# dafyddstephenson/ucla-roms

Hardware: AMD Instinct MI355X
Metric: grid-cell-updates/sec (higher is better)
Workload: dtype f64; 1 GPU; C3: basin 1024x1024x100, NONLIN+SPLIT EOS, T+S, LMD KPP/BKPP/RIMIX/NONLOCAL, dt=300s, ndtfast=60 (nfast=82); NT=2, nfast=82, parallelism=domain decomposition 1x1, halo_transport=none (single rank), fast_exchange_interval=1, exchange_order=none (single rank), s2d_window=True, comm_bootstrap=none (single rank)

## Files before the change

### include/roms_gpu.h

```cpp
#ifndef ROMS_GPU_H
#define ROMS_GPU_H

#ifdef __cplusplus
extern "C" {
#endif

#define ROMS_GPU_ABI_VERSION 22
#define ROMS_MAX_FAST 288

typedef struct roms_dims {
  int Lm, Mm, N, NT;
  int LLm, MMm;
  int np_xi, np_eta, inode, jnode;
  int iSW_corn, jSW_corn;
  int ew_periodic, ns_periodic;
  int west_exchng, east_exchng, south_exchng, north_exchng;
} roms_dims;

#define ROMS_LMD_MIXING   1
#define ROMS_LMD_KPP      2
#define ROMS_LMD_BKPP     4
#define ROMS_LMD_RIMIX    8
#define ROMS_LMD_CONVEC   16
#define ROMS_LMD_NONLOCAL 32
#define ROMS_LMD_ALL      63
#define ROMS_LMD_ICELAND  47
#define ROMS_LMD_DDMIX    64

typedef struct roms_cfg {
  int nonlin_eos;
// ... 101 lines not shown
} roms_case;
int roms_gpu_init_case(const roms_case *c, int device, roms_tlev *t);
int roms_gpu_init_case_comm(const roms_case *c, int np_xi, int np_eta, void *comm, int device, roms_tlev *t);

int roms_gpu_comm_unique_id(void *id128);
int roms_gpu_comm_create(const void *id128, int nranks, int rank, int device, void **comm);
int roms_gpu_comm_create_local(int group, int nranks, int rank, void **comm);
typedef int (*roms_host_allgather_fn)(void *ctx, const void *send, long nbytes, void *recv);
int roms_gpu_comm_create_host(int nranks, int rank, int device, roms_host_allgather_fn allgather, void *ctx,
                              void **comm);
int roms_gpu_comm_destroy(void *comm);
int roms_gpu_halo_transport(void);
int roms_gpu_halo_exchanges(long *per_step, int *fast_interval);
int roms_gpu_halo_overlap(void);
int roms_gpu_s2d_window(void);
#define ROMS_COLPATH_SEG 1
#define ROMS_COLPATH_GLOBAL 2
int roms_gpu_column_path(void);
int roms_gpu_kpp_lean(void);
int roms_gpu_vgrid(void);
int roms_gpu_vgrid2(void);
int roms_gpu_vgrid_check(long out[3]);
int roms_gpu_tracer_pair(long launches[2]);
int roms_gpu_horizontal_path(int out[8]);
int roms_gpu_selftest_zero_fill(long n, int chunks, long *bad);
int roms_gpu_halo_plan(int Lm, int Mm, int np_xi, int np_eta, int inode, int jnode, int ew_periodic,
                       int ns_periodic, int peer[8], long count[8], int strip[4]);
long roms_gpu_halo_map(int Lm, int Mm, int np_xi, int np_eta, int inode, int jnode, int ew_periodic,
                       int ns_periodic, int dir, int unpack, int *i, int *j, long cap);
long roms_gpu_halo_map_wide(int Lm, int Mm, int np_xi, int np_eta, int inode, int jnode, int ew_periodic,
                            int ns_periodic, int width, int dir, int unpack, int *i, int *j, long cap);

#define ROMS_FRC_SURFACE 1
#define ROMS_FRC_BRY     2
int roms_gpu_frc_record(int field_id, int slot, double rec_time, const double *data);
int roms_gpu_frc_interp(double modtime, int kinds);
int roms_gpu_frc_clock(double start_time, int on);
int roms_gpu_set_tide_data(int ntides, const double *ftide, const double *pot_re, const double *pot_im,
                           const double *ztide_re, const double *ztide_im, const double *utide_re,
                           const double *utide_im, const double *vtide_re, const double *vtide_im);
int roms_gpu_set_tides(double time);

#define ROMS_WRT_Z    1
#define ROMS_WRT_UB   2
#define ROMS_WRT_VB   4
#define ROMS_WRT_U    8
// ... 40 lines not shown
```

### ucla-roms_amd/csrc/k_common.h

```cpp
#pragma once
#include "roms_dev.h"
#include <type_traits>

namespace roms {

constexpr unsigned kBufOff = 0x80000000u;
struct BufF64 {
  __amdgpu_buffer_rsrc_t r;
  __device__ __forceinline__ explicit BufF64(const double* p, long n = 0)
      : r(__builtin_amdgcn_make_buffer_rsrc(const_cast<double*>(p), (short)0,
                                            n > 0 ? (int)(unsigned)(n * 8) : (int)0x7fffffff, 0x00020000)) {}
  __device__ __forceinline__ double ld(unsigned vb, unsigned sb) const {
    return __builtin_bit_cast(double, __builtin_amdgcn_raw_buffer_load_b64(r, (int)vb, (int)sb, 0));
  }
  __device__ __forceinline__ void st(double v, unsigned vb, unsigned sb) const {
    __builtin_amdgcn_raw_buffer_store_b64(__builtin_bit_cast(__attribute__((ext_vector_type(2))) int, v), r, (int)vb,
                                          (int)sb, 0);
  }
};

constexpr int kUVW = kBX + 4, kUVH = kBY + 4, kUVN = kUVW * kUVH;

struct ColLds {
  double* p;
// ... 173 lines not shown
  const double Fl = a.fu(m, j);
  if (upstream) {
    const double cm = el[1] - el[0], c0 = el[2] - el[1];
    return 0.5 * (a.t(m, j) + a.t(m - 1, j)) * Fl - 0.1666666666666666 * (cm * fmax0(Fl) + c0 * fmin0(Fl));
  }
  const double gm = 0.5 * (el[1] + el[0]), g0 = 0.5 * (el[2] + el[1]);
  return 0.5 * (a.t(m, j) + a.t(m - 1, j) - 0.3333333333333333 * (g0 - gm)) * Fl;
}
template <class A>
__device__ __forceinline__ double tracer_fe(const Bounds& b, const A& a, int i, int m, bool upstream) {
  const int lo = b.south_edge ? b.jstr : -1000000, hi = b.north_edge ? b.jend + 1 : 1000000;
  double el[3];
  for (int q = 0; q < 3; q++) {
    const int p = iclamp(m - 1 + q, lo, hi);
    el[q] = (a.t(i, p) - a.t(i, p - 1)) * a.vm(i, p);
  }
  const double Fl = a.fv(i, m);
  if (upstream) {
    const double cm = el[1] - el[0], c0 = el[2] - el[1];
    return 0.5 * (a.t(i, m) + a.t(i, m - 1)) * Fl - 0.1666666666666666 * (cm * fmax0(Fl) + c0 * fmin0(Fl));
  }
  const double gm = 0.5 * (el[1] + el[0]), g0 = 0.5 * (el[2] + el[1]);
  return 0.5 * (a.t(i, m) + a.t(i, m - 1) - 0.3333333333333333 * (g0 - gm)) * Fl;
}

struct TracerWin {
  double T[kUVN], UM[kUVN], VM[kUVN], FU[kUVN], FV[kUVN];
};
__device__ __forceinline__ void tracer_win_fill(const Bounds& b, const Fields& F, TracerWin& W, int ib, int jb,
                                                long kk, const double* T) {
  for (int q = threadIdx.x + kBX * threadIdx.y; q < kUVN; q += kBX * kBY) {
    const int i = ib + q % kUVW, j = jb + q / kUVW;
    if (i < -1 || i > b.Lm + 2 || j < -1 || j > b.Mm + 2) continue;
    const long o = IJ(b, i, j);
    if (T) {
      W.T[q] = T[o + kk];
    } else {
      W.UM[q] = F.umask[o];
      W.VM[q] = F.vmask[o];
      W.FU[q] = F.FlxU[o + kk];
      W.FV[q] = F.FlxV[o + kk];
    }
  }
}

struct UVBounds {
// ... 293 lines not shown
```

### ucla-roms_amd/csrc/k_pre_step3d.hip

```cpp
#include "k_colseg.h"

namespace roms {

struct PreCoef {
  double dtau, cf_stp, cf_bak;
};

__global__ void __launch_bounds__(256) k_pre_tracer_h(Dev d, Range R, PreCoef c, int nstp, int nnew, int nrhs) {
  const uint3 bI = xcd_tile();
  __shared__ TracerWin W;
  const Bounds& b = d.b;
  const Fields& F = d.f;
  const int k = 1 + (int)bI.z, indx = 3 - nstp;
  const int i0 = tile_i0(R.i0) + (int)bI.x * kBX, j0 = R.j0 + (int)bI.y * kBY;
  const int ib = i0 - 2, jb = j0 - 2;
  const long kk = (long)(k - 1) * b.n2;
  tracer_win_fill(b, F, W, ib, jb, kk, nullptr);
  const int i = i0 + (int)threadIdx.x, j = j0 + (int)threadIdx.y;
  const bool act = i >= R.i0 && i <= R.i1 && j <= R.j1;
  const long ij = IJ(b, i, j), o = ij + kk;
  double hb = 0.0;
  if (act) {
    double hf;
    hz_bak_fwd(d, i, j, k, 0.5 * c.dtau, hb, hf);
// ... 96 lines not shown
    const double FlxDiv = cff * pm * pn * (fu1 - fu0 + fv1 - fv0 + we1 + wi1 - we0 - wi0);
    hb = hzo + FlxDiv;
    const double hf = hzo - FlxDiv;
    F.c2[o] = hf;
    F.c3[o] = hb;
  }
  if (!in) return;
  const double hz = hzo;
#pragma unroll
  for (int t = 0; t < NTT; t++) {
    const int itrc = t + 1;
    const AccTL a{W.T[t], W.UM, W.VM, W.FU, W.FV, ib, jb};
    double FX0 = tracer_fx(b, a, i, j, false), FX1 = tracer_fx(b, a, i + 1, j, false);
    double FE0 = tracer_fe(b, a, i, j, false), FE1 = tracer_fe(b, a, i, j + 1, false);
    if (d.p.nriv > 0) {
      river_tracer_flux(d, 0, i, j, k, itrc, FX0); river_tracer_flux(d, 0, i + 1, j, k, itrc, FX1);
      river_tracer_flux(d, 1, i, j, k, itrc, FE0); river_tracer_flux(d, 1, i, j + 1, k, itrc, FE1);
    }
    const long tb = (long)t * 3 * b.n3;
    const double tsk = ts[t];
    F.t[(long)(nnew - 1) * b.n3 + tb + o] =
        hb * (c.cf_stp * tsk + c.cf_bak * ti[t]) - c.dtau * pm * pn * (FX1 - FX0 + FE1 - FE0);
    F.t[(long)(indx - 1) * b.n3 + tb + o] = hz * tsk;
  }
}

template <class C>
__global__ void __launch_bounds__(64) k_pre_tracer_v(Dev d, Range R, PreCoef c, int nnew, int nrhs) {
  ROMS_IJC_OR_RETURN(R)
  col_lds_poison<C>(2, d.b.N);
  const Bounds& b = d.b;
  const Fields& F = d.f;
  const int N = b.N;
  const long n2 = b.n2, ij = IJ(b, i, j);
  const double* __restrict__ Hz = F.Hz + ij;
  const double* __restrict__ We = F.We + ij;
  const double* __restrict__ Wi = F.Wi + ij;
  const C A = ColMake<C>::at(d, 0, (int)bI.z, ij), B = ColMake<C>::at(d, 1, (int)bI.z, ij);
  const double* __restrict__ Hf = F.c2 + ij;
  auto hfwd = [&](int k) { return Hf[(long)(k - 1) * n2]; };
  {
    const int itrc = 1 + (int)bI.z;
    const long tb = (long)(itrc - 1) * 3 * b.n3;
    const double* __restrict__ Tr = F.t + (long)(nrhs - 1) * b.n3 + tb + ij;
    double* __restrict__ Tn = F.t + (long)(nnew - 1) * b.n3 + tb + ij;
    tracer_spline_lds(N, n2, Hz, Tr, We, A, B);
// ... 786 lines not shown
void setup_column_kernels_t(size_t bytes);
void setup_column_kernels_uv1(size_t bytes);
bool setup_column_kernels(int N) {
  const size_t bytes = col_lds_bytes(2, N);
  if (bytes > 160 * 1024) return false;
  if (bytes > 64 * 1024) {
    (void)hipFuncSetAttribute((const void*)k_pre_tracer_v<ColLds>, hipFuncAttributeMaxDynamicSharedMemorySize,
                              (int)bytes);
    (void)hipFuncSetAttribute((const void*)k_pre_uv<ColLds>, hipFuncAttributeMaxDynamicSharedMemorySize, (int)bytes);
    setup_column_kernels_t(bytes);
    setup_column_kernels_uv1(bytes);
  }
  return true;
}

static thread_local long t_pair_count[2] = {0, 0};
long t_pair_launches(int bit, long add, bool reset) {
  if (reset) t_pair_count[0] = t_pair_count[1] = 0;
  long& c = t_pair_count[bit == kTPairCor ? 1 : 0];
  c += add;
  return c;
}

double pre_step3d_dtau(const Dev& d, const Tlev& t) {
  const double AM3_crv = 1.0 / 6.0;
  return t.iic == t.forw_start ? 0.5 * d.p.dt : d.p.dt * (1.0 - AM3_crv);
}

void launch_pre_step3d(const Dev& d, hipStream_t s, const Tlev& t, bool uv_done, bool hb_done) {
  const Bounds& b = d.b;
  PreCoef c;
  const double AM3_crv = 1.0 / 6.0;
  if (t.iic == t.forw_start) { c.dtau = 0.5 * d.p.dt; c.cf_stp = 1.0; c.cf_bak = 0.0; }
  else { c.dtau = d.p.dt * (1.0 - AM3_crv); c.cf_stp = 0.5 + AM3_crv; c.cf_bak = 0.5 - AM3_crv; }
  c.dtau = pre_step3d_dtau(d, t);
  hb_done = hb_done && d.p.hoist && b.NT <= 2;
  Range RI{b.istr, b.iend, b.jstr, b.jend};
  Range RH{b.istr - 1, b.iend, b.jstr - 1, b.jend};
  auto horiz_tiles = [&](const Range& rh) {
    const dim3 gh = grid3_of(rh, b.N), bh(kBX, kBY);
    if (d.p.hoist && b.NT == 2 && hb_done)
      hipLaunchKernelGGL((k_pre_tracer_h1<2, true>), gh, bh, 0, s, d, rh, c, t.nstp, t.nnew, t.nrhs);
    else if (d.p.hoist && b.NT == 2)
      hipLaunchKernelGGL((k_pre_tracer_h1<2, false>), gh, bh, 0, s, d, rh, c, t.nstp, t.nnew, t.nrhs);
    else if (d.p.hoist && b.NT == 1 && hb_done)
      hipLaunchKernelGGL((k_pre_tracer_h1<1, true>), gh, bh, 0, s, d, rh, c, t.nstp, t.nnew, t.nrhs);
    else if (d.p.hoist && b.NT == 1)
      hipLaunchKernelGGL((k_pre_tracer_h1<1, false>), gh, bh, 0, s, d, rh, c, t.nstp, t.nnew, t.nrhs);
    else
      hipLaunchKernelGGL(k_pre_tracer_h, gh, bh, 0, s, d, rh, c, t.nstp, t.nnew, t.nrhs);
  };
  {
    int jA = 0, jB = -1;
    if (d.p.hoist &&
        launch_tracer_strip(d, s, RH, 1, false, hb_done, t.nnew, t.nrhs, c.dtau, c.cf_stp, c.cf_bak, t.nstp, jA, jB)) {
      if (jA > RH.j0) horiz_tiles(Range{RH.i0, RH.i1, RH.j0, jA - 1});
      if (jB < RH.j1) horiz_tiles(Range{RH.i0, RH.i1, jB + 1, RH.j1});
    } else {
      horiz_tiles(RH);
    }
  }
  dim3 gt = gridc_of(RI);
  gt.z = b.NT;
  if (d.p.colseg && d.p.seg_buf && (d.p.t_pair & kTPairPre) && b.NT == 2 && b.nTS == 2) {
// ... 47 lines not shown
```

### ucla-roms_amd/csrc/k_step3d_t.hip

```cpp
#include "k_colseg.h"

namespace roms {

__global__ void __launch_bounds__(256) k_step3d_t_h(Dev d, Range R, int nnew, int nrhs, int up) {
  const uint3 bI = xcd_tile();
  __shared__ TracerWin W;
  const Bounds& b = d.b;
  const Fields& F = d.f;
  const int k = 1 + (int)bI.z;
  const int i0 = tile_i0(R.i0) + (int)bI.x * kBX, j0 = R.j0 + (int)bI.y * kBY;
  const int ib = i0 - 2, jb = j0 - 2;
  const long kk = (long)(k - 1) * b.n2;
  tracer_win_fill(b, F, W, ib, jb, kk, nullptr);
  const int i = i0 + (int)threadIdx.x, j = j0 + (int)threadIdx.y;
  const bool act = i >= R.i0 && i <= R.i1 && j <= R.j1;
  const long ij = IJ(b, i, j), o = ij + kk;
  const AccTL a{W.T, W.UM, W.VM, W.FU, W.FV, ib, jb};
  for (int itrc = 1; itrc <= b.NT; itrc++) {
    const long tb = (long)(itrc - 1) * 3 * b.n3;
    const double* Tr = F.t + (long)(nrhs - 1) * b.n3 + tb;
    __syncthreads();
    tracer_win_fill(b, F, W, ib, jb, kk, Tr);
    __syncthreads();
    if (!act) continue;
// ... 49 lines not shown
  for (int t = 0; t < NTT; t++) tn[t] = F.t[(long)(nnew - 1) * b.n3 + (long)t * 3 * b.n3 + o];
#pragma unroll
  for (int r = 0; r < NR; r++) {
    const int q = tid + r * kBX * kBY;
    if (q < NW) {
      W.UM[q] = wUM[r]; W.VM[q] = wVM[r]; W.FU[q] = wFU[r]; W.FV[q] = wFV[r];
#pragma unroll
      for (int t = 0; t < NTT; t++) W.T[t][q] = wT[t][r];
    }
  }
  __syncthreads();
  if (!act) return;
#pragma unroll
  for (int t = 0; t < NTT; t++) {
    const int itrc = t + 1;
    const AccTL a{W.T[t], W.UM, W.VM, W.FU, W.FV, ib, jb};
    double FX0 = tracer_fx(b, a, i, j, true), FX1 = tracer_fx(b, a, i + 1, j, true);
    double FE0 = tracer_fe(b, a, i, j, true), FE1 = tracer_fe(b, a, i, j + 1, true);
    if (d.p.nriv > 0) {
      river_tracer_flux(d, 0, i, j, k, itrc, FX0); river_tracer_flux(d, 0, i + 1, j, k, itrc, FX1);
      river_tracer_flux(d, 1, i, j, k, itrc, FE0); river_tracer_flux(d, 1, i, j + 1, k, itrc, FE1);
    }
    F.t[(long)(nnew - 1) * b.n3 + (long)t * 3 * b.n3 + o] = tn[t] - d.p.dt * pm * pn * (FX1 - FX0 + FE1 - FE0);
  }
}

template <class C, bool ISO = false>
__global__ void __launch_bounds__(64) k_step3d_t_v(Dev d, Range R, int nnew, int nrhs) {
  ROMS_IJC_OR_RETURN(R)
  col_lds_poison<C>(2, d.b.N);
  const Bounds& b = d.b;
  const Fields& F = d.f;
  const Params& P = d.p;
  const int N = b.N;
  const double dt = P.dt;
  const long n2 = b.n2, ij = IJ(b, i, j);
  const double rm = F.rmask[ij];
  const double* __restrict__ Hz = F.Hz + ij;
  const C A = ColMake<C>::at(d, 0, (int)bI.z, ij), B = ColMake<C>::at(d, 1, (int)bI.z, ij);
  {
    const int itrc = 1 + (int)bI.z;
    const double* __restrict__ Tr = F.t + (long)(nrhs - 1) * b.n3 + (long)(itrc - 1) * 3 * b.n3 + ij;
    double* __restrict__ Tn = F.t + (long)(nnew - 1) * b.n3 + (long)(itrc - 1) * 3 * b.n3 + ij;
    const double stf = F.stflx[ij + (long)(itrc - 1) * n2];
    tracer_spline_lds(N, n2, Hz, Tr, F.We + ij, A, B);
    A[N] = 0.0;
// ... 540 lines not shown
                            (int)bytes);
  (void)hipFuncSetAttribute((const void*)k_step3d_t_v<ColLds, true>, hipFuncAttributeMaxDynamicSharedMemorySize,
                            (int)bytes);
}

void launch_step3d_t(const Dev& d, hipStream_t s, const Tlev& t, bool exchange) {
  const Bounds& b = d.b;
  Range R{b.istr, b.iend, b.jstr, b.jend};
  if (d.p.iso) {
    hipLaunchKernelGGL(k_step3d_t_h, grid3_of(R, b.N), dim3(kBX, kBY), 0, s, d, R, t.nnew, t.nrhs, 0);
    for (int itrc = 1; itrc <= b.NT; itrc++) launch_iso_tracer(d, s, t, itrc);
    dim3 gt = gridc_of(R);
    gt.z = b.NT;
    if (d.f.colscr)
      hipLaunchKernelGGL((k_step3d_t_v<ColGlb, true>), gt, dim3(kCX), 0, s, d, R, t.nnew, t.nrhs);
    else
      hipLaunchKernelGGL((k_step3d_t_v<ColLds, true>), gt, dim3(kCX), col_lds_bytes(2, b.N), s, d, R, t.nnew, t.nrhs);
    for (int itrc = 1; itrc <= b.NT; itrc++) launch_t3dbc(d, s, t, itrc);
    launch_exchange_tracers(d, s, t.nnew);
    return;
  }
  auto h_tiles = [&](const Range& r) {
    const dim3 gh = grid3_of(r, b.N), bh(kBX, kBY);
    if (d.p.hoist && b.NT == 2)
      hipLaunchKernelGGL(k_step3d_t_h1<2>, gh, bh, 0, s, d, r, t.nnew, t.nrhs);
    else if (d.p.hoist && b.NT == 1)
      hipLaunchKernelGGL(k_step3d_t_h1<1>, gh, bh, 0, s, d, r, t.nnew, t.nrhs);
    else
      hipLaunchKernelGGL(k_step3d_t_h, gh, bh, 0, s, d, r, t.nnew, t.nrhs, 1);
  };
  auto run = [&](const Range& r) {
    int jA = 0, jB = -1;
    if (d.p.hoist && launch_tracer_strip(d, s, r, 0, true, false, t.nnew, t.nrhs, 0.0, 0.0, 0.0, 0, jA, jB)) {
      if (jA > r.j0) h_tiles(Range{r.i0, r.i1, r.j0, jA - 1});
      if (jB < r.j1) h_tiles(Range{r.i0, r.i1, jB + 1, r.j1});
    } else {
      h_tiles(r);
    }
    dim3 gt = gridc_of(r);
    gt.z = b.NT;
    if (d.p.colseg) {
      ktimer_mark(s, kTimedStep3dTSeg, 0);
      if (d.p.seg_buf && (d.p.t_pair & kTPairCor) && b.NT == 2 && b.nTS == 2) {
        hipLaunchKernelGGL(k_step3d_t_segb_pair, seg_grid_of(r, 1), dim3(kCX, seg_waves(b.N)), 0, s, d, r, t.nnew, t.nrhs);
        t_pair_launches(kTPairCor, 1);
      } else if (d.p.seg_buf)
        hipLaunchKernelGGL(k_step3d_t_segb, seg_grid_of(r, b.NT), dim3(kCX, seg_waves(b.N)), 0, s, d, r, t.nnew, t.nrhs);
// ... 202 lines not shown
```

### ucla-roms_amd/csrc/roms_dev.h

```cpp
#pragma once
#include <hip/hip_runtime.h>
#include <cstddef>
#include <cstdint>

namespace roms {

constexpr int kMaxFast = 288;
constexpr int kRowAlign = 16;
constexpr int kAlignOff = 14;

struct Bounds {
  int Lm, Mm, N, NT, nTS, nx2;
  long n2, n3, n3w;
  int gx;
  int istr, iend, jstr, jend;
  int istrU, istrR, iendR, jstrV, jstrR, jendR;
  int istrE, iendE, jstrE, jendE;
  int west_edge, east_edge, south_edge, north_edge;
  int ew_periodic, ns_periodic;
  int west_exch, east_exch, south_exch, north_exch;
};

struct Params {
  int nonlin_eos, salinity, lmd, uv_vis2, ts_dif2;
// ... 12 lines not shown
  int seg_order;
  int seg_xg;
  int s2d_fold;
  int hoist;
  int chain_dirz;
  int prs_fuse_uv;
  int : 32;
  int prs_buf;
  int prs_strip;
  int t_strip;
  int visc_stg;
  int t3dmix_stg;
  int kpp_ty;
  int uv1_lds;
  int omega_seg;
  int omega_cw;
  int p_in_rho;
  int omega_hb;
  int preuv_lds;
  int seg_jrows;
  int seg_buf;
  int vgrid2;
  int t_pair;
  int reserved_[6];
  int s2d_k;
  int uv2e_nc, uv2e_nf;
  int npip;
  int nriv, nrivf;
  int curvgrid;
  int obc;
  short kpp_lean;
  short kpp_fckeep;
  short vgrid;
  short vg;
  double ubind;
  double dt, dtfast, g, rho0, vonKar, qp2, gamma2, hc;
  double rdrg, Zob, Tcoef, T0, Scoef, S0;
  double Akv_bak, Akt_bak[2];
};
static_assert(offsetof(Params, s2d_k) == 196 && offsetof(Params, ubind) == 240 && sizeof(Params) == 384,
              "Params: no member from s2d_k on may move");

struct Fields {
  double *h, *hinv, *f, *fomn, *pm, *pn, *dm_r, *dn_r, *dm_u, *dn_u, *dm_v, *dn_v, *dm_p, *dn_p,
      *pmon_u, *pnom_v, *rmask, *pmask, *umask, *vmask;
  double *dndx, *dmde;
  double* ptide;
// ... 54 lines not shown
}
__host__ __device__ __forceinline__ long IJL(const Bounds& b, int i, int j, int l) {
  return IJ(b, i, j) + (long)(l - 1) * b.n2;
}
__host__ __device__ __forceinline__ long IJKL(const Bounds& b, int i, int j, int k, int l) {
  return IJ(b, i, j) + (long)(k - 1) * b.n2 + (long)(l - 1) * b.n3;
}
__host__ __device__ __forceinline__ long TIDX(const Bounds& b, int i, int j, int k, int l, int itrc) {
  return IJKL(b, i, j, k, l) + (long)(itrc - 1) * 3 * b.n3;
}

__device__ __forceinline__ double fmax0(double a) { return a > 0.0 ? a : 0.0; }
__device__ __forceinline__ double fmin0(double a) { return a < 0.0 ? a : 0.0; }
__device__ __forceinline__ double dmax(double a, double b) { return a > b ? a : b; }
__device__ __forceinline__ double dmin(double a, double b) { return a < b ? a : b; }
__device__ __forceinline__ int iclamp(int x, int lo, int hi) { return x < lo ? lo : (x > hi ? hi : x); }

constexpr int kVgRho = 1, kVgKppExt = 2, kVgKppInt = 4, kVgHuv = 8, kVgAll = 15;
constexpr int kVgDefault = kVgRho | kVgKppExt | kVgHuv;
constexpr int kVg2Omega = 1, kVg2Huv1 = 2, kVg2Uv2 = 4, kVg2Visc = 8, kVg2T3dmix = 16, kVg2All = 31, kVg2Shift = 8;
constexpr int kVg2Default = kVg2All;
constexpr int kTPairPre = 1, kTPairCor = 2, kTPairAll = 3;
constexpr int kTPairDefault = kTPairAll;
struct VGrid {
  const double *Cs_w, *Cs_r;
  double z, h, hinv, hc, ds;
  int N;
  __device__ __forceinline__ double zw0() const { return -h; }
  __device__ __forceinline__ double zw1(int k, double csw) const {
    const double cff_w = hc * ds * (double)(k - N);
    return z + (z + h) * (cff_w + csw * h) * hinv;
  }
  __device__ __forceinline__ double zr(int k, double csr) const {
    const double cff_r = hc * ds * ((double)(k - N) - 0.5);
    return z + (z + h) * (cff_r + csr * h) * hinv;
  }
  __device__ __forceinline__ double zw(int k, double csw) const { return k == 0 ? zw0() : zw1(k, csw); }
  __device__ __forceinline__ double zw1(int k) const { return zw1(k, Cs_w[k]); }
  __device__ __forceinline__ double zr(int k) const { return zr(k, Cs_r[k]); }
};
__device__ __forceinline__ double vg_zw(const VGrid& g, int k) { return k == 0 ? g.zw0() : g.zw1(k); }
__device__ __forceinline__ double vg_zr(const VGrid& g, int k) { return g.zr(k); }
__device__ __forceinline__ double vg_hz(const VGrid& g, int k) { return g.zw1(k) - vg_zw(g, k - 1); }
__device__ __forceinline__ VGrid vg_make(const Dev& d, double z, double h, double hinv) {
  return VGrid{d.f.Cs_w, d.f.Cs_r, z, h, hinv, d.p.hc, 1.0 / (double)d.b.N, d.b.N};
}
// ... 131 lines not shown
  edges();
  rim_fork(d, s, L);
  run(Range{R.i0 + 2, R.i1 - 2, R.j0 + 2, R.j1 - 2});
  rim_join(d, s);
}
bool tracer_exch_list(const Dev& d, int tlev, ExchList& L);
void launch_exchange_tracers(const Dev& d, hipStream_t s, int tlev);
bool setup_column_kernels(int N);
void setup_uv1_seg();
void setup_pre_uv_seg();
inline size_t col_smem_bytes(const Dev& d, int nslots) {
  return d.f.colscr ? 0 : (size_t)nslots * (d.b.N + 1) * 64 * sizeof(double);
}
void launch_set_depth(const Dev& d, hipStream_t s, const Tlev& t, bool exchange = true, bool last = false);
void launch_set_huv(const Dev& d, hipStream_t s, const Tlev& t, bool store_huv = true);
void launch_vgrid_check(const Dev& d, hipStream_t s, unsigned long long* cnt);
void launch_set_huv1(const Dev& d, hipStream_t s, const Tlev& t);
bool launch_omega(const Dev& d, hipStream_t s, const Tlev& t, double hcff = 0.0);
void setup_omega_seg();
bool omega_takes_seg(const Dev& d, int width);
int s2d_edge_mode(const Dev& d);
int s2d_edge_modes_taken(bool reset = false);
long t_pair_launches(int bit, long add = 0, bool reset = false);
bool prsgrd_takes_strips(const Dev& d, bool with_uv, int& jA, int& jB, int& nstrip);
double pre_step3d_dtau(const Dev& d, const Tlev& t);
void launch_rho_eos(const Dev& d, hipStream_t s, const Tlev& t, int tidx);
void launch_prsgrd(const Dev& d, hipStream_t s, const Tlev& t, int uv_up = -1, bool p_ready = false);
bool launch_tracer_strip(const Dev& d, hipStream_t s, const Range& R, int mode, bool up, bool hb_done, int nnew,
                         int nrhs, double dtau, double cf_stp, double cf_bak, int nstp, int& jA, int& jB);
bool p_in_rho(const Dev& d);
bool prsgrd_can_fuse_uv(const Dev& d);
void launch_pre_step3d(const Dev& d, hipStream_t s, const Tlev& t, bool uv_done = false, bool hb_done = false);
void launch_step3d_uv1(const Dev& d, hipStream_t s, const Tlev& t, bool uv_done = false);
void launch_visc3d(const Dev& d, hipStream_t s, const Tlev& t);
void launch_step2d(const Dev& d, hipStream_t s, const Tlev& t, const double* w1, const double* w2);
void launch_step3d_uv2(const Dev& d, hipStream_t s, const Tlev& t);
void launch_step3d_t(const Dev& d, hipStream_t s, const Tlev& t, bool exchange = true);
void launch_t3dmix(const Dev& d, hipStream_t s, const Tlev& t);
void launch_u3dbc(const Dev& d, hipStream_t s, const Tlev& t);
void launch_river_s2d(const Dev& d, hipStream_t s, int knew);
void launch_bulk_flux(const Dev& d, hipStream_t s, int nrhs);
void launch_river_uv(const Dev& d, hipStream_t s, int nnew, int pred);
void launch_v3dbc(const Dev& d, hipStream_t s, const Tlev& t);
void launch_t3dbc(const Dev& d, hipStream_t s, const Tlev& t, int itrc);
void launch_diag(const Dev& d, hipStream_t s, const Tlev& t, double* out);
void launch_swr_frac(const Dev& d, hipStream_t s);
// ... 9 lines not shown
```

### ucla-roms_amd/csrc/roms_shim.cpp

```cpp
#include <hip/hip_runtime.h>

#include <algorithm>
#include <cmath>
#include <cstdlib>
#include <cstdio>
#include <cstring>
#include <map>
#include <string>
#include <vector>

#include "../../include/roms_gpu.h"
#include "halo.h"
#include "host_init.h"
#include "roms_dev.h"
#include "shim_state.h"

using namespace roms;

namespace {

struct FieldDesc {
  double* d = nullptr;
  long count = 0;
  long hcount = 0;
// ... 3 lines not shown
};

struct Ctx {
  bool inited = false;
  Dev d{};
  hipStream_t s = nullptr;
  FieldDesc f[ROMS_NFIELDS];
  std::vector<double*> scratch;
  roms_dims dims{};
  roms_cfg cfg{};
  double w1[kMaxFast], w2[kMaxFast];
  double area = 0.0, volume = 0.0;
  bool have_volume = false;
  long riv_maxidx = 0;
  bool have_swr = false;
  long graph_frc_gen = 0;
  int rho_slot = 0;
  bool hzuv_env = false;
  bool hzuv_valid = true;
  bool rho_reuse = true;
  bool vgrid_valid = false;
  bool akt_same = false;
  int t_pair_cfg = 0;
  std::string err;
  std::map<long, hipGraphExec_t> graphs;
  bool use_graphs = true;
  double* h_diag = nullptr;
  double* d_diag = nullptr;
  Halo halo;
  int timed = -1;
  std::vector<hipEvent_t> ev;
  size_t nev = 0;
  long kcount = 0;
  bool guard = false;
  std::map<double*, double*> guard_base;
  double* arena = nullptr;
  long arena_n = 0, arena_used = 0;
  double* small = nullptr;
  long small_n = 0;
  long off = 0;
  Bounds hb{};
  double* stage = nullptr;
  long stage_n = 0;
  long step_exch = 0;
};
thread_local Ctx g;
// ... 14 lines not shown
  if (node == 0) len -= off / 2;
  if (node == np - 1) len -= (off + 1) / 2;
}
int min_rank_extent(int LL, int np) {
  int mn = LL, len, sw;
  for (int node : {0, np - 1}) {
    rank_extent(LL, np, node, len, sw);
    mn = len < mn ? len : mn;
  }
  if (np > 2) {
    rank_extent(LL, np, 1, len, sw);
    mn = len < mn ? len : mn;
  }
  return mn;
}

void drop_graphs() {
  for (auto& kv : g.graphs) (void)hipGraphExecDestroy(kv.second);
  g.graphs.clear();
}
void vg_set(bool valid) {
  g.vgrid_valid = valid;
  g.d.p.vg = valid ? (short)(g.d.p.vgrid | (g.d.p.vgrid2 << kVg2Shift)) : (short)0;
}
void akt_set(bool same) {
  g.akt_same = same;
  g.d.p.t_pair = same ? g.t_pair_cfg : 0;
}
void akt_lmd_done() {
  const Params& P = g.d.p;
  akt_set(g.cfg.lmd_mixing && !P.lmd_ddmix && g.d.b.nTS == 2 &&
          std::memcmp(&P.Akt_bak[0], &P.Akt_bak[1], sizeof(double)) == 0);
}
void vg_host_write(int id) {
  if (id == ROMS_Akt) akt_set(false);
  if (id != ROMS_Hz && id != ROMS_z_r && id != ROMS_z_w && id != ROMS_h && id != ROMS_hinv && id != ROMS_Cs_w &&
      id != ROMS_Cs_r)
    return;
  if (g.vgrid_valid && !g.graphs.empty()) {
    (void)hipStreamSynchronize(g.s);
    drop_graphs();
  }
  vg_set(false);
}

#define CHECK_HIP(x)                                                                  \
// ... 574 lines not shown
  P.omega_hb = !env_off("ROMS_GPU_OMEGA_HB");
  P.omega_seg = !env_off("ROMS_GPU_OMEGA_SEG");
  {
    const int v = env_int("ROMS_GPU_OMEGA_CW", dims->N > 63 ? 16 : 64, 0, 1 << 30);
    P.omega_cw = v == 32 || v == 64 ? v : 16;
  }
  P.preuv_lds = !env_off("ROMS_GPU_PREUV_LDS");
  P.visc_stg = !env_off("ROMS_GPU_VISC_STG");
  P.t3dmix_stg = !env_off("ROMS_GPU_T3DMIX_STG");
  {
    const int v = env_int("ROMS_GPU_KPP_TY", 4, 0, 43);
    P.kpp_ty = v == 0 || v == 2 || v == 8 || v == 43 ? v : 4;
  }
  P.kpp_lean = (short)env_int("ROMS_GPU_KPP_LEAN", 7, 0, 7);
  P.kpp_fckeep = (short)env_int("ROMS_GPU_KPP_FCKEEP", kKppFcKeepMax, 1, kKppFcKeepMax);
  P.vgrid = (short)env_int("ROMS_GPU_VGRID", kVgDefault, 0, kVgAll);
  P.vgrid2 = env_int("ROMS_GPU_VGRID2", kVg2Default, 0, kVg2All);
  P.vg = 0;
  g.vgrid_valid = false;
  g.t_pair_cfg = env_int("ROMS_GPU_T_PAIR", kTPairDefault, 0, kTPairAll);
  P.t_pair = 0;
  g.akt_same = false;
  (void)t_pair_launches(0, 0, true);
  P.hoist = !env_off("ROMS_GPU_HOIST");
  P.prs_buf = !env_off("ROMS_GPU_PRS_BUF");
  P.prs_strip = !env_off("ROMS_GPU_PRS_STRIP");
  P.t_strip = env_on("ROMS_GPU_T_STRIP");
  P.seg_buf = !env_off("ROMS_GPU_SEG_BUF");
  P.seg_jrows = env_int("ROMS_GPU_SEG_JROWS", kSegJMax < 2 ? kSegJMax : 2, 1, kSegJMax);
  bool col_global = (size_t)2 * (dims->N + 1) * kCX * sizeof(double) > 64 * 1024;
  if (env_on("ROMS_GPU_COL_GLOBAL")) col_global = true;
  if (env_off("ROMS_GPU_COL_GLOBAL")) col_global = false;
  setup_uv1_seg();
  setup_pre_uv_seg();
  setup_omega_seg();
  if (!col_global && !setup_column_kernels(dims->N)) {
    g.err = "roms_gpu_init: N too large for the LDS column kernels (2*(N+1)*512 B > 160 KB)";
    return -2;
  }
  CHECK_HIP(hipStreamCreateWithFlags(&g.s, hipStreamNonBlocking));
  g.guard = env_on("ROMS_GPU_GUARD");
  const Bounds& b = g.d.b;
  auto field = [&](int id) -> int {
    const long n = field_count(id, b);
    double* p = nullptr;
    CHECK_HIP(dev_alloc(p, n));
// ... 212 lines not shown
  REQUIRE_INIT_NOJOIN();
  return g.d.w2.base ? 1 : 0;
}

int roms_gpu_column_path(void) {
  REQUIRE_INIT_NOJOIN();
  return (g.d.p.colseg ? ROMS_COLPATH_SEG : 0) | (g.d.f.colscr ? ROMS_COLPATH_GLOBAL : 0);
}

int roms_gpu_vgrid(void) {
  REQUIRE_INIT_NOJOIN();
  return g.d.p.vgrid + (g.vgrid_valid ? 256 : 0);
}

int roms_gpu_vgrid2(void) {
  REQUIRE_INIT_NOJOIN();
  return g.d.p.vgrid2 + (g.vgrid_valid ? 256 : 0);
}

int roms_gpu_tracer_pair(long launches[2]) {
  REQUIRE_INIT_NOJOIN();
  if (launches) { launches[0] = t_pair_launches(kTPairPre); launches[1] = t_pair_launches(kTPairCor); }
  return g.t_pair_cfg + (g.akt_same ? 256 : 0);
}

int roms_gpu_vgrid_check(long out[3]) {
  REQUIRE_INIT_RO();
  if (!out) { g.err = "roms_gpu_vgrid_check: null argument"; return -1; }
  unsigned long long* cnt = (unsigned long long*)shim_scratch_small(3);
  if (!cnt) { g.err = "roms_gpu_vgrid_check: out of device memory"; return -2; }
  CHECK_HIP(hipMemsetAsync(cnt, 0, 3 * sizeof(unsigned long long), g.s));
  launch_vgrid_check(g.d, g.s, cnt);
  unsigned long long h[3] = {0, 0, 0};
  CHECK_HIP(copy_on(h, cnt, sizeof(h), hipMemcpyDeviceToHost, g.s));
  for (int q = 0; q < 3; q++) out[q] = (long)h[q];
  return post_launch();
}

int roms_gpu_kpp_lean(void) {
  REQUIRE_INIT_NOJOIN();
  return g.d.p.kpp_lean + 256 * g.d.p.kpp_fckeep;
}

int roms_gpu_horizontal_path(int out[8]) {
  REQUIRE_INIT_NOJOIN();
  if (!out) { g.err = "roms_gpu_horizontal_path: null argument"; return -1; }
// ... 579 lines not shown
```

### ucla-roms_amd/romsgpu/__init__.py

```python
import ctypes
import os

import numpy as np

_HERE = os.path.dirname(os.path.abspath(__file__))
_PKG = os.path.dirname(_HERE)
LIB_PATH = os.environ.get("ROMS_GPU_LIB") or os.path.join(_PKG, "libromsgpu.so")
MAX_FAST = 288

FIELDS = ["h", "hinv", "f", "fomn", "pm", "pn", "dm_r", "dn_r", "dm_u", "dn_u", "dm_v", "dn_v", "dm_p", "dn_p",
          "pmon_u", "pnom_v", "rmask", "pmask", "umask", "vmask", "Cs_w", "Cs_r",
          "zeta", "ubar", "vbar", "u", "v", "t", "FlxU", "FlxV", "We", "Wi", "Hz", "Hz_u", "Hz_v", "z_r", "z_w",
          "rufrc", "rvfrc", "rhoA", "rhoS", "r_D", "Zt_avg1", "DU_avg1", "DV_avg1", "DU_avg2", "DV_avg2",
          "DU_avg_bak", "DV_avg_bak", "rho", "rho1", "qp1", "bvf", "Akv", "Akt", "visc2_r", "visc2_p", "diff2",
          "hbls", "hbbl", "ghat", "swr_frac", "sustr", "svstr", "stflx", "srflx", "swflx", "ru", "rv"] + \
         ["%s_%s" % (v, e) for v in ("zeta", "ubar", "vbar", "u", "v", "t") for e in ("west", "east", "south", "north")] + \
         ["dndx", "dmde", "ptide", "uwnd", "vwnd", "tair", "qair", "prate", "swrad", "lwrad", "sustr_r", "svstr_r"]
FIELD_ID = {n: i for i, n in enumerate(FIELDS)}
CASE_FILAMENT, CASE_BASIN, CASE_PIPES, CASE_RIVERS = 0, 1, 2, 3
LMD_MIXING, LMD_KPP, LMD_BKPP, LMD_RIMIX, LMD_CONVEC, LMD_NONLOCAL = 1, 2, 4, 8, 16, 32
LMD_DDMIX = 64
LMD_ALL = 63
LMD_ICELAND = 47

# ... 452 lines not shown
        return bool(self.L.roms_gpu_s2d_window())

    def kpp_lean(self):
        r = self.L.roms_gpu_kpp_lean()
        self._chk(min(r, 0), "kpp_lean")
        return r % 256, r // 256

    def vgrid(self):
        r = self.L.roms_gpu_vgrid()
        self._chk(min(r, 0), "vgrid")
        return r % 256, bool(r // 256)

    def vgrid2(self):
        r = self.L.roms_gpu_vgrid2()
        self._chk(min(r, 0), "vgrid2")
        return r % 256, bool(r // 256)

    def tracer_pair(self):
        n = (ctypes.c_long * 2)(0, 0)
        r = self.L.roms_gpu_tracer_pair(n)
        self._chk(min(r, 0), "tracer_pair")
        return r % 256, bool(r // 256), (n[0], n[1])

    def vgrid_mismatch(self):
        out = (ctypes.c_long * 3)()
        self._chk(self.L.roms_gpu_vgrid_check(out), "vgrid_check")
        return out[0], out[1], out[2]

    def column_path(self):
        r = self.L.roms_gpu_column_path()
        self._chk(min(r, 0), "column_path")
        return bool(r & 1), bool(r & 2)

    def horizontal_path(self):
        out = (ctypes.c_int * 8)()
        self._chk(self.L.roms_gpu_horizontal_path(out), "horizontal_path")
        return {"edges": out[0], "strips": (out[2], out[3], out[4]) if out[1] else None, "omega_seg": bool(out[5])}

    def fast_step_edge_modes(self):
        out = (ctypes.c_int * 8)()
        self._chk(self.L.roms_gpu_horizontal_path(out), "horizontal_path")
        return {m for m in range(3) if out[6] >> m & 1}

    def halo_exchanges(self):
        n, k = ctypes.c_long(), ctypes.c_int()
        self._chk(self.L.roms_gpu_halo_exchanges(ctypes.byref(n), ctypes.byref(k)), "halo_exchanges")
# ... 49 lines not shown
```

Before: 2.470 billion cell-updates/s.

## Stage tracer horizontal advection stencils in LDS with k-marching kernels

Adds new tracer advection kernels for the predictor and corrector steps. Each block marches down the vertical levels and stages FlxU, FlxV and both tracers for a tile plus a 2-cell halo in shared memory, with the next level prefetched into registers. The predictor variant can also recompute Hz on the fly from the vertical grid instead of loading it. This aims to cut redundant global loads of the 4th-order stencil neighbours. In exchange it adds two barriers per level and shared-memory pressure that may limit occupancy. The new path is enabled by default through an env-controlled flag, with a launch counter and query API.

Result: faster. 2.508 billion cell-updates/s (median of 6 runs) (+1.5%).

```diff
diff --git a/include/roms_gpu.h b/include/roms_gpu.h
--- a/include/roms_gpu.h
+++ b/include/roms_gpu.h
@@ -5,7 +5,7 @@
 extern "C" {
 #endif
 
-#define ROMS_GPU_ABI_VERSION 22
+#define ROMS_GPU_ABI_VERSION 23
 #define ROMS_MAX_FAST 288
 
 typedef struct roms_dims {
@@ -153,6 +153,7 @@
 int roms_gpu_vgrid2(void);
 int roms_gpu_vgrid_check(long out[3]);
 int roms_gpu_tracer_pair(long launches[2]);
+int roms_gpu_tracer_hstg(long launches[3]);
 int roms_gpu_horizontal_path(int out[8]);
 int roms_gpu_selftest_zero_fill(long n, int chunks, long *bad);
 int roms_gpu_halo_plan(int Lm, int Mm, int np_xi, int np_eta, int inode, int jnode, int ew_periodic,
diff --git a/ucla-roms_amd/csrc/k_common.h b/ucla-roms_amd/csrc/k_common.h
--- a/ucla-roms_amd/csrc/k_common.h
+++ b/ucla-roms_amd/csrc/k_common.h
@@ -219,6 +219,107 @@
   }
   const double gm = 0.5 * (el[1] + el[0]), g0 = 0.5 * (el[2] + el[1]);
   return 0.5 * (a.t(i, m) + a.t(i, m - 1) - 0.3333333333333333 * (g0 - gm)) * Fl;
+}
+
+#ifndef ROMS_T_HSTG_ROWS
+#define ROMS_T_HSTG_ROWS 8
+#endif
+constexpr int kTSWaves = 4;
+constexpr int kTSY = ROMS_T_HSTG_ROWS, kTSB = kBX * kTSY;
+constexpr int kTSN = kUVW * (kTSY + 4);
+constexpr int kTSR = (kTSN + kTSB - 1) / kTSB;
+inline dim3 grid_tstg(const Range& r) {
+  int ni = r.i1 - tile_i0(r.i0) + 1, nj = r.j1 - r.j0 + 1;
+  if (ni < 1) ni = 1;
+  if (nj < 1) nj = 1;
+  return dim3((ni + kBX - 1) / kBX, (nj + kTSY - 1) / kTSY, 1);
+}
+struct TracerStg {
+  double L[4][kTSN];
+  __device__ __forceinline__ void put(int tid, const double (&w)[4][kTSR]) {
+#pragma unroll
+    for (int r = 0; r < kTSR; r++) {
+      const int q = tid + r * kTSB;
+      if (q < kTSN) {
+#pragma unroll
+        for (int f = 0; f < 4; f++) L[f][q] = w[f][r];
+      }
+    }
+  }
+};
+struct TracerStgLd {
+  unsigned o[kTSR];
+  __device__ __forceinline__ TracerStgLd(const Bounds& b, int ib, int jb, int tid) {
+#pragma unroll
+    for (int r = 0; r < kTSR; r++) {
+      const int q = tid + r * kTSB;
+      const int i = ib + q % kUVW, j = jb + q / kUVW;
+      const bool ok = q < kTSN && i >= -1 && i <= b.Lm + 2 && j >= -1 && j <= b.Mm + 2;
+      o[r] = ok ? (unsigned)IJ(b, i, j) * 8u : kBufOff;
+    }
+  }
+  __device__ __forceinline__ void ld(const BufF64& FU, const BufF64& FV, const BufF64& T0, const BufF64& T1, unsigned lev,
+                                     double (&w)[4][kTSR]) const {
+#pragma unroll
+    for (int r = 0; r < kTSR; r++) {
+      w[0][r] = FU.ld(o[r], lev);
+      w[1][r] = FV.ld(o[r], lev);
+      w[2][r] = T0.ld(o[r], lev);
+      w[3][r] = T1.ld(o[r], lev);
+    }
+  }
+};
+
+__device__ __forceinline__ double tracer_face(double el0, double el1, double el2, double tm, double tm1, double Fl,
+                                              bool upstream) {
+  if (upstream) {
+    const double cm = el1 - el0, c0 = el2 - el1;
+    return 0.5 * (tm + tm1) * Fl - 0.1666666666666666 * (cm * fmax0(Fl) + c0 * fmin0(Fl));
+  }
+  const double gm = 0.5 * (el1 + el0), g0 = 0.5 * (el2 + el1);
+  return 0.5 * (tm + tm1 - 0.3333333333333333 * (g0 - gm)) * Fl;
+}
+__device__ __forceinline__ void tracer_face_pair(int lo, int hi, int c, const double (&T)[5], const double (&M)[4],
+                                                 double F0, double F1, bool upstream, double& X0, double& X1) {
+  double E[4];
+#pragma unroll
+  for (int q = 0; q < 4; q++) E[q] = (T[q + 1] - T[q]) * M[q];
+  const double a0 = c - 1 < lo ? E[1] : E[0];
+  const double b2 = c + 2 > hi ? E[2] : E[3];
+  X0 = tracer_face(a0, E[1], E[2], T[2], T[1], F0, upstream);
+  X1 = tracer_face(E[1], E[2], b2, T[3], T[2], F1, upstream);
+}
+struct TracerStgMask {
+  double UM[4], VM[4];
+  __device__ __forceinline__ TracerStgMask(const Bounds& b, const Fields& F, long ij) {
+#pragma unroll
+    for (int q = 0; q < 4; q++) {
+      UM[q] = F.umask[ij - 1 + q];
+      VM[q] = F.vmask[ij + (q - 1) * (long)b.nx2];
+    }
+  }
+};
+struct TracerStgFlx {
+  double FU[2], FV[2];
+  __device__ __forceinline__ TracerStgFlx(const TracerStg& W, int cw) {
+    FU[0] = W.L[0][cw]; FU[1] = W.L[0][cw + 1];
+    FV[0] = W.L[1][cw]; FV[1] = W.L[1][cw + kUVW];
+  }
+};
+__device__ __forceinline__ void tracer_stg_fluxes(const Bounds& b, const TracerStg& W, const TracerStgMask& M,
+                                                  const TracerStgFlx& S, int t, int cw, int i, int j, bool upstream,
+                                                  double& FX0, double& FX1, double& FE0, double& FE1) {
+  const double* T = W.L[2 + t];
+  double TX[5], TY[5];
+#pragma unroll
+  for (int q = 0; q < 5; q++) {
+    TX[q] = T[cw - 2 + q];
+    TY[q] = q == 2 ? TX[2] : T[cw + (q - 2) * kUVW];
+  }
+  tracer_face_pair(b.west_edge ? b.istr : -1000000, b.east_edge ? b.iend + 1 : 1000000, i, TX, M.UM, S.FU[0], S.FU[1],
+                   upstream, FX0, FX1);
+  tracer_face_pair(b.south_edge ? b.jstr : -1000000, b.north_edge ? b.jend + 1 : 1000000, j, TY, M.VM, S.FV[0], S.FV[1],
+                   upstream, FE0, FE1);
 }
 
 struct TracerWin {
diff --git a/ucla-roms_amd/csrc/k_pre_step3d.hip b/ucla-roms_amd/csrc/k_pre_step3d.hip
--- a/ucla-roms_amd/csrc/k_pre_step3d.hip
+++ b/ucla-roms_amd/csrc/k_pre_step3d.hip
@@ -142,6 +142,107 @@
     F.t[(long)(nnew - 1) * b.n3 + tb + o] =
         hb * (c.cf_stp * tsk + c.cf_bak * ti[t]) - c.dtau * pm * pn * (FX1 - FX0 + FE1 - FE0);
     F.t[(long)(indx - 1) * b.n3 + tb + o] = hz * tsk;
+  }
+}
+
+template <bool kHB, bool VG>
+__global__ void __launch_bounds__(kTSB, kTSWaves) k_pre_tracer_stg(Dev d, Range R, PreCoef c, int nstp, int nnew, int nrhs) {
+  const uint3 bI = xcd_tile();
+  __shared__ TracerStg W;
+  const Bounds& b = d.b;
+  const Fields& F = d.f;
+  const int N = b.N, indx = 3 - nstp;
+  const int i0 = tile_i0(R.i0) + (int)bI.x * kBX, j0 = R.j0 + (int)bI.y * kTSY;
+  const int ib = i0 - 2, jb = j0 - 2;
+  const long n2 = b.n2;
+  const int tid = threadIdx.x + kBX * threadIdx.y;
+  const TracerStgLd E(b, ib, jb, tid);
+  const long ts = 3 * b.n3;
+  const BufF64 FU(F.FlxU), FV(F.FlxV);
+  const BufF64 Tr0(F.t + (long)(nrhs - 1) * b.n3), Tr1(F.t + (long)(nrhs - 1) * b.n3 + ts);
+  const BufF64 Ts0(F.t + (long)(nstp - 1) * b.n3), Ts1(F.t + (long)(nstp - 1) * b.n3 + ts);
+  const BufF64 Ti0(F.t + (long)(indx - 1) * b.n3), Ti1(F.t + (long)(indx - 1) * b.n3 + ts);
+  const BufF64 Tn0(F.t + (long)(nnew - 1) * b.n3), Tn1(F.t + (long)(nnew - 1) * b.n3 + ts);
+  const BufF64 C2(F.c2), C3(F.c3), Hz(F.Hz), We(F.We), Wi(F.Wi);
+  const unsigned ls = (unsigned)n2 * 8u;
+  double w[4][kTSR];
+  E.ld(FU, FV, Tr0, Tr1, 0u, w);
+  const int i = i0 + (int)threadIdx.x, j = j0 + (int)threadIdx.y;
+  const bool act = i >= R.i0 && i <= R.i1 && j <= R.j1;
+  const bool in = act && i >= b.istr && j >= b.jstr;
+  const bool formed = kHB && in;
+  const long ij = act ? IJ(b, i, j) : IJ(b, R.i0, R.j0);
+  const unsigned vo = (unsigned)ij * 8u;
+  const unsigned vin = in ? vo : kBufOff, vhb = act && !formed ? vo : kBufOff;
+  double we0 = 0.0, wi0 = 0.0;
+  if (!formed) { we0 = F.We[ij]; wi0 = F.Wi[ij]; }
+  double gz = 0.0, gh = 0.0, gi = 0.0, gw = 0.0, csw = 0.0;
+  if constexpr (VG) {
+    gz = F.z_sd[ij]; gh = F.h[ij]; gi = F.hinv[ij];
+    gw = -gh;
+    csw = F.Cs_w[1];
+  }
+  const double pm = F.pm[ij], pn = F.pn[ij];
+  const TracerStgMask M(b, F, ij);
+  bool rx0 = false, rx1 = false, re0 = false, re1 = false;
+  if (d.p.nriv > 0 && in) {
+    rx0 = fabs(F.riv_uflx[ij]) > 1e-3; rx1 = fabs(F.riv_uflx[ij + 1]) > 1e-3;
+    re0 = fabs(F.riv_vflx[ij]) > 1e-3; re1 = fabs(F.riv_vflx[ij + b.nx2]) > 1e-3;
+  }
+  const bool riv = rx0 || rx1 || re0 || re1;
+  const int cw = (int)threadIdx.x + 2 + ((int)threadIdx.y + 2) * kUVW;
+  unsigned lev = 0u;
+  for (int k = 1; k <= N; k++, lev += ls) {
+    double x1, y1 = 0.0;
+    if (formed) {
+      x1 = C3.ld(vo, lev);
+    } else {
+      x1 = We.ld(vo, lev + ls); y1 = Wi.ld(vo, lev + ls);
+    }
+    double hz;
+    if constexpr (!VG) hz = Hz.ld(vo, lev);
+    const double tsk0 = Ts0.ld(vo, lev), tsk1 = Ts1.ld(vo, lev), tik0 = Ti0.ld(vo, lev), tik1 = Ti1.ld(vo, lev);
+    const double cs = csw;
+    if constexpr (VG) csw = F.Cs_w[min(k + 1, N)];
+    if (k > 1) __syncthreads();
+    W.put(tid, w);
+    if (k < N) E.ld(FU, FV, Tr0, Tr1, lev + ls, w);
+    if constexpr (VG) {
+      const double z = vg_make(d, gz, gh, gi).zw1(k, cs);
+      hz = z - gw;
+      gw = z;
+    }
+    __syncthreads();
+    const TracerStgFlx S(W, cw);
+    double hb = x1;
+    if (!formed) {
+      const double fu0 = S.FU[0], fu1 = S.FU[1], fv0 = S.FV[0], fv1 = S.FV[1];
+      const double we1 = x1, wi1 = y1;
+      const double cff = 0.5 * c.dtau;
+      const double FlxDiv = cff * pm * pn * (fu1 - fu0 + fv1 - fv0 + we1 + wi1 - we0 - wi0);
+      hb = hz + FlxDiv;
+      const double hf = hz - FlxDiv;
+      C2.st(hf, vhb, lev);
+      C3.st(hb, vhb, lev);
+      we0 = we1; wi0 = wi1;
+    }
+#pragma unroll
+    for (int t = 0; t < 2; t++) {
+      const int itrc = t + 1;
+      double FX0, FX1, FE0, FE1;
+      tracer_stg_fluxes(b, W, M, S, t, cw, i, j, false, FX0, FX1, FE0, FE1);
+      if (riv) {
+        int kr = k, ir = i, jr = j;
+        __asm__ volatile("" : "+s"(kr), "+v"(ir), "+v"(jr));
+        if (rx0) river_tracer_flux(d, 0, ir, jr, kr, itrc, FX0);
+        if (rx1) river_tracer_flux(d, 0, ir + 1, jr, kr, itrc, FX1);
+        if (re0) river_tracer_flux(d, 1, ir, jr, kr, itrc, FE0);
+        if (re1) river_tracer_flux(d, 1, ir, jr + 1, kr, itrc, FE1);
+      }
+      const double tsk = t == 0 ? tsk0 : tsk1, tik = t == 0 ? tik0 : tik1;
+      (t == 0 ? Tn0 : Tn1).st(hb * (c.cf_stp * tsk + c.cf_bak * tik) - c.dtau * pm * pn * (FX1 - FX0 + FE1 - FE0), vin, lev);
+      (t == 0 ? Ti0 : Ti1).st(hz * tsk, vin, lev);
+    }
   }
 }
 
@@ -974,6 +1075,14 @@
   return c;
 }
 
+static thread_local long t_hstg_count[3] = {0, 0, 0};
+long t_hstg_launches(int bit, long add, bool reset) {
+  if (reset) t_hstg_count[0] = t_hstg_count[1] = t_hstg_count[2] = 0;
+  long& c = t_hstg_count[bit == kTHstgCor ? 1 : bit == kTHstgHz ? 2 : 0];
+  c += add;
+  return c;
+}
+
 double pre_step3d_dtau(const Dev& d, const Tlev& t) {
   const double AM3_crv = 1.0 / 6.0;
   return t.iic == t.forw_start ? 0.5 * d.p.dt : d.p.dt * (1.0 - AM3_crv);
@@ -991,7 +1100,20 @@
   Range RH{b.istr - 1, b.iend, b.jstr - 1, b.jend};
   auto horiz_tiles = [&](const Range& rh) {
     const dim3 gh = grid3_of(rh, b.N), bh(kBX, kBY);
-    if (d.p.hoist && b.NT == 2 && hb_done)
+    if (d.p.hoist && b.NT == 2 && (d.p.t_hstg & kTHstgPre)) {
+      const bool vg = (d.p.t_hstg & kTHstgHz) != 0;
+      const dim3 gs = grid_tstg(rh), bs(kBX, kTSY);
+      if (hb_done && vg)
+        hipLaunchKernelGGL((k_pre_tracer_stg<true, true>), gs, bs, 0, s, d, rh, c, t.nstp, t.nnew, t.nrhs);
+      else if (hb_done)
+        hipLaunchKernelGGL((k_pre_tracer_stg<true, false>), gs, bs, 0, s, d, rh, c, t.nstp, t.nnew, t.nrhs);
+      else if (vg)
+        hipLaunchKernelGGL((k_pre_tracer_stg<false, true>), gs, bs, 0, s, d, rh, c, t.nstp, t.nnew, t.nrhs);
+      else
+        hipLaunchKernelGGL((k_pre_tracer_stg<false, false>), gs, bs, 0, s, d, rh, c, t.nstp, t.nnew, t.nrhs);
+      t_hstg_launches(kTHstgPre, 1);
+      if (vg) t_hstg_launches(kTHstgHz, 1);
+    } else if (d.p.hoist && b.NT == 2 && hb_done)
       hipLaunchKernelGGL((k_pre_tracer_h1<2, true>), gh, bh, 0, s, d, rh, c, t.nstp, t.nnew, t.nrhs);
     else if (d.p.hoist && b.NT == 2)
       hipLaunchKernelGGL((k_pre_tracer_h1<2, false>), gh, bh, 0, s, d, rh, c, t.nstp, t.nnew, t.nrhs);
diff --git a/ucla-roms_amd/csrc/k_step3d_t.hip b/ucla-roms_amd/csrc/k_step3d_t.hip
--- a/ucla-roms_amd/csrc/k_step3d_t.hip
+++ b/ucla-roms_amd/csrc/k_step3d_t.hip
@@ -95,6 +95,63 @@
       river_tracer_flux(d, 1, i, j, k, itrc, FE0); river_tracer_flux(d, 1, i, j + 1, k, itrc, FE1);
     }
     F.t[(long)(nnew - 1) * b.n3 + (long)t * 3 * b.n3 + o] = tn[t] - d.p.dt * pm * pn * (FX1 - FX0 + FE1 - FE0);
+  }
+}
+
+__global__ void __launch_bounds__(kTSB, kTSWaves) k_step3d_t_stg(Dev d, Range R, int nnew, int nrhs) {
+  const uint3 bI = xcd_tile();
+  __shared__ TracerStg W;
+  const Bounds& b = d.b;
+  const Fields& F = d.f;
+  const int N = b.N;
+  const int i0 = tile_i0(R.i0) + (int)bI.x * kBX, j0 = R.j0 + (int)bI.y * kTSY;
+  const int ib = i0 - 2, jb = j0 - 2;
+  const long n2 = b.n2;
+  const int tid = threadIdx.x + kBX * threadIdx.y;
+  const TracerStgLd E(b, ib, jb, tid);
+  const long ts = 3 * b.n3;
+  const BufF64 FU(F.FlxU), FV(F.FlxV);
+  const BufF64 Tr0(F.t + (long)(nrhs - 1) * b.n3), Tr1(F.t + (long)(nrhs - 1) * b.n3 + ts);
+  const BufF64 Tn0(F.t + (long)(nnew - 1) * b.n3), Tn1(F.t + (long)(nnew - 1) * b.n3 + ts);
+  const unsigned ls = (unsigned)n2 * 8u;
+  double w[4][kTSR];
+  E.ld(FU, FV, Tr0, Tr1, 0u, w);
+  const int i = i0 + (int)threadIdx.x, j = j0 + (int)threadIdx.y;
+  const bool act = i >= R.i0 && i <= R.i1 && j <= R.j1;
+  const long ij = act ? IJ(b, i, j) : IJ(b, R.i0, R.j0);
+  const unsigned vo = (unsigned)ij * 8u, vs = act ? vo : kBufOff;
+  const double pm = F.pm[ij], pn = F.pn[ij];
+  const TracerStgMask M(b, F, ij);
+  bool rx0 = false, rx1 = false, re0 = false, re1 = false;
+  if (d.p.nriv > 0 && act) {
+    rx0 = fabs(F.riv_uflx[ij]) > 1e-3; rx1 = fabs(F.riv_uflx[ij + 1]) > 1e-3;
+    re0 = fabs(F.riv_vflx[ij]) > 1e-3; re1 = fabs(F.riv_vflx[ij + b.nx2]) > 1e-3;
+  }
+  const bool riv = rx0 || rx1 || re0 || re1;
+  const int cw = (int)threadIdx.x + 2 + ((int)threadIdx.y + 2) * kUVW;
+  unsigned lev = 0u;
+  for (int k = 1; k <= N; k++, lev += ls) {
+    const double tn0 = Tn0.ld(vo, lev), tn1 = Tn1.ld(vo, lev);
+    if (k > 1) __syncthreads();
+    W.put(tid, w);
+    if (k < N) E.ld(FU, FV, Tr0, Tr1, lev + ls, w);
+    __syncthreads();
+    const TracerStgFlx S(W, cw);
+#pragma unroll
+    for (int t = 0; t < 2; t++) {
+      const int itrc = t + 1;
+      double FX0, FX1, FE0, FE1;
+      tracer_stg_fluxes(b, W, M, S, t, cw, i, j, true, FX0, FX1, FE0, FE1);
+      if (riv) {
+        int kr = k, ir = i, jr = j;
+        __asm__ volatile("" : "+s"(kr), "+v"(ir), "+v"(jr));
+        if (rx0) river_tracer_flux(d, 0, ir, jr, kr, itrc, FX0);
+        if (rx1) river_tracer_flux(d, 0, ir + 1, jr, kr, itrc, FX1);
+        if (re0) river_tracer_flux(d, 1, ir, jr, kr, itrc, FE0);
+        if (re1) river_tracer_flux(d, 1, ir, jr + 1, kr, itrc, FE1);
+      }
+      (t == 0 ? Tn0 : Tn1).st((t == 0 ? tn0 : tn1) - d.p.dt * pm * pn * (FX1 - FX0 + FE1 - FE0), vs, lev);
+    }
   }
 }
 
@@ -681,7 +738,10 @@
   }
   auto h_tiles = [&](const Range& r) {
     const dim3 gh = grid3_of(r, b.N), bh(kBX, kBY);
-    if (d.p.hoist && b.NT == 2)
+    if (d.p.hoist && b.NT == 2 && (d.p.t_hstg & kTHstgCor)) {
+      hipLaunchKernelGGL(k_step3d_t_stg, grid_tstg(r), dim3(kBX, kTSY), 0, s, d, r, t.nnew, t.nrhs);
+      t_hstg_launches(kTHstgCor, 1);
+    } else if (d.p.hoist && b.NT == 2)
       hipLaunchKernelGGL(k_step3d_t_h1<2>, gh, bh, 0, s, d, r, t.nnew, t.nrhs);
     else if (d.p.hoist && b.NT == 1)
       hipLaunchKernelGGL(k_step3d_t_h1<1>, gh, bh, 0, s, d, r, t.nnew, t.nrhs);
diff --git a/ucla-roms_amd/csrc/roms_dev.h b/ucla-roms_amd/csrc/roms_dev.h
--- a/ucla-roms_amd/csrc/roms_dev.h
+++ b/ucla-roms_amd/csrc/roms_dev.h
@@ -58,7 +58,8 @@
   int seg_buf;
   int vgrid2;
   int t_pair;
-  int reserved_[6];
+  int t_hstg;
+  int reserved_[5];
   int s2d_k;
   int uv2e_nc, uv2e_nf;
   int npip;
@@ -159,6 +160,8 @@
 constexpr int kVg2Default = kVg2All;
 constexpr int kTPairPre = 1, kTPairCor = 2, kTPairAll = 3;
 constexpr int kTPairDefault = kTPairAll;
+constexpr int kTHstgPre = 1, kTHstgCor = 2, kTHstgHz = 4, kTHstgAll = 7;
+constexpr int kTHstgDefault = kTHstgAll, kTHstgDefaultCol = kTHstgCor;
 struct VGrid {
   const double *Cs_w, *Cs_r;
   double z, h, hinv, hc, ds;
@@ -336,6 +339,7 @@
 int s2d_edge_mode(const Dev& d);
 int s2d_edge_modes_taken(bool reset = false);
 long t_pair_launches(int bit, long add = 0, bool reset = false);
+long t_hstg_launches(int bit, long add = 0, bool reset = false);
 bool prsgrd_takes_strips(const Dev& d, bool with_uv, int& jA, int& jB, int& nstrip);
 double pre_step3d_dtau(const Dev& d, const Tlev& t);
 void launch_rho_eos(const Dev& d, hipStream_t s, const Tlev& t, int tidx);
diff --git a/ucla-roms_amd/csrc/roms_shim.cpp b/ucla-roms_amd/csrc/roms_shim.cpp
--- a/ucla-roms_amd/csrc/roms_shim.cpp
+++ b/ucla-roms_amd/csrc/roms_shim.cpp
@@ -49,6 +49,7 @@
   bool vgrid_valid = false;
   bool akt_same = false;
   int t_pair_cfg = 0;
+  int t_hstg_cfg = 0;
   std::string err;
   std::map<long, hipGraphExec_t> graphs;
   bool use_graphs = true;
@@ -109,6 +110,7 @@
 void vg_set(bool valid) {
   g.vgrid_valid = valid;
   g.d.p.vg = valid ? (short)(g.d.p.vgrid | (g.d.p.vgrid2 << kVg2Shift)) : (short)0;
+  g.d.p.t_hstg = valid ? g.t_hstg_cfg : (g.t_hstg_cfg & ~kTHstgHz);
 }
 void akt_set(bool same) {
   g.akt_same = same;
@@ -729,6 +731,9 @@
   P.t_pair = 0;
   g.akt_same = false;
   (void)t_pair_launches(0, 0, true);
+  g.t_hstg_cfg = env_int("ROMS_GPU_T_HSTG", P.colseg ? kTHstgDefault : kTHstgDefaultCol, 0, kTHstgAll);
+  P.t_hstg = g.t_hstg_cfg & ~kTHstgHz;
+  (void)t_hstg_launches(0, 0, true);
   P.hoist = !env_off("ROMS_GPU_HOIST");
   P.prs_buf = !env_off("ROMS_GPU_PRS_BUF");
   P.prs_strip = !env_off("ROMS_GPU_PRS_STRIP");
@@ -987,6 +992,16 @@
   REQUIRE_INIT_NOJOIN();
   if (launches) { launches[0] = t_pair_launches(kTPairPre); launches[1] = t_pair_launches(kTPairCor); }
   return g.t_pair_cfg + (g.akt_same ? 256 : 0);
+}
+
+int roms_gpu_tracer_hstg(long launches[3]) {
+  REQUIRE_INIT_NOJOIN();
+  if (launches) {
+    launches[0] = t_hstg_launches(kTHstgPre);
+    launches[1] = t_hstg_launches(kTHstgCor);
+    launches[2] = t_hstg_launches(kTHstgHz);
+  }
+  return g.t_hstg_cfg + (g.vgrid_valid ? 256 : 0);
 }
 
 int roms_gpu_vgrid_check(long out[3]) {
diff --git a/ucla-roms_amd/romsgpu/__init__.py b/ucla-roms_amd/romsgpu/__init__.py
--- a/ucla-roms_amd/romsgpu/__init__.py
+++ b/ucla-roms_amd/romsgpu/__init__.py
@@ -498,6 +498,12 @@
         self._chk(min(r, 0), "tracer_pair")
         return r % 256, bool(r // 256), (n[0], n[1])
 
+    def tracer_hstg(self):
+        n = (ctypes.c_long * 3)(0, 0, 0)
+        r = self.L.roms_gpu_tracer_hstg(n)
+        self._chk(min(r, 0), "tracer_hstg")
+        return r % 256, bool(r // 256), (n[0], n[1], n[2])
+
     def vgrid_mismatch(self):
         out = (ctypes.c_long * 3)()
         self._chk(self.L.roms_gpu_vgrid_check(out), "vgrid_check")
```
